# lh3/bfc

Measured on AMD Instinct MI355X. Metric: M k-mers/s counted (bloom+htab) on 150 bp reads, higher is better.
Workload: dtype u64

## Files before the change

bfc_amd/csrc/bfcg_bloom3.hip:

```cpp
#include <hip/hip_runtime.h>
#include <stdint.h>
#include <stdlib.h>
#include "kmer_dev.h"
#include "bfcg_internal.h"
#include "bfcg_dev.h"

using namespace bfcg;

#define B3_UND 0x40000000u
#define B3_SEEN16 0x8000u
#define B3_COLD_NR 8
#define B3_WALK_U 4
template <int BT, int PF, bool COLD>
__global__ __launch_bounds__(BT, PF <= 2 ? 8 : 6) void k_bloom3(KParams P, BloomArgs A)
{
	extern __shared__ __attribute__((aligned(16))) unsigned char smem[];
	__shared__ uint32_t s_list_n, s_ovf, s_pool_off, s_emit_n, s_fs_used, s_wb_n, s_pad3[2];
	const uint32_t f = blockIdx.x;
	const bool ho_log = A.ho_stride != 0;
	if (batch_poisoned(A)) { if (ho_log && threadIdx.x == 0) A.ho_mark[f] = A.ho_cur[f]; return; }
	uint32_t rs, n;
	region_list(A, f, rs, n);
	if (n == 0) { if (threadIdx.x == 0) { if (ho_log) A.ho_mark[f] = A.ho_cur[f]; else if (A.agg_cnt) A.agg_cnt[f] = 0; } return; }
	uint32_t ho_cur0 = 0;
	unsigned long long *ho_base;
	if (ho_log) {
		ho_cur0 = A.ho_cur[f];
		if (ho_cur0 + n > A.ho_stride) {
			if (threadIdx.x == 0) { atomicAdd(&A.stats[(size_t)(f & (ST_SLOTS - 1)) * ST_N + ST_ERR_POOL], 1ULL); A.ho_mark[f] = ho_cur0; }
			return;
		}
		ho_base = A.ho + (uint64_t)f * A.ho_stride + ho_cur0;
	} else ho_base = reinterpret_cast<unsigned long long *>(A.stream_out) + rs;
	A.stats += (size_t)(f & (ST_SLOTS - 1)) * ST_N;
	const uint32_t region_dw = 16u << P.R;
	unsigned char *sp = smem;
	unsigned int *region = reinterpret_cast<unsigned int *>(sp); sp += (size_t)region_dw * 4;
	const uint32_t nblk = 1u << P.R;
	unsigned int *bcnt = reinterpret_cast<unsigned int *>(sp), *boff = bcnt + nblk;
	if (COLD) sp += (size_t)(2 * nblk + 4) * 4;
	unsigned int *fs = reinterpret_cast<unsigned int *>(sp); if (!COLD) sp += (size_t)P.fs_cap * 4;
	unsigned int *la = reinterpret_cast<unsigned int *>(sp); sp += (size_t)P.list_cap * 4;
	unsigned int *lb = reinterpret_cast<unsigned int *>(sp); sp += (size_t)P.list_cap * 4;
	unsigned short *lc = reinterpret_cast<unsigned short *>(sp); sp += (size_t)P.list_cap * 2;
	unsigned short *ord = reinterpret_cast<unsigned short *>(sp);
	const uint32_t fs_mask = P.fs_cap - 1;
	const uint32_t *recs = A.recs + (uint64_t)rs * 3;
	unsigned int *g_region = reinterpret_cast<unsigned int *>(A.bloom) + (uint64_t)f * region_dw;
	const uint32_t imp = (P.f_base + f) >> P.F2;
	const Dec3 D = dec3_geom(P);
	const int tid = threadIdx.x, lane = tid & 63;
	const uint32_t mask_a = (1u << D.a) - 1u, imp_sh = D.n ? imp << D.lo : 0u, sh_up = D.lo + D.n;
#ifdef BFCG_MEASURE
	const bool timing = BFCG_ABL(P, 64) && tid == 0;
	long long tq[7] = {0, 0, 0, 0, 0, 0, 0};
	long long tc[7] = {0, 0, 0, 0, 0, 0, 0};
	if (timing) tq[0] = clock64();
#define B3_TC(i) do { if (timing) tc[i] = clock64(); } while (0)
#else
#define B3_TC(i) do { } while (0)
#endif
	auto addr3 = [&](uint32_t d0, uint32_t d1) -> uint32_t {
		const uint32_t y0d = d0 & mask_a, upper = y0d >> D.up;
		const uint32_t y0lo = D.n ? (y0d & D.lowmask) | imp_sh | (upper << sh_up) : y0d;
		const uint32_t y1lo = __builtin_amdgcn_alignbit(d1, d0, D.a) & D.mk32;
		const uint32_t hh = upper | (((y0lo - y1lo) ^ y1lo) << D.sh_x);
		uint32_t h2 = (hh >> 9) & 511u;
		h2 |= (uint32_t)((h2 & 31u) == 0);
		return (y0d & D.rmask) | ((hh & 511u) << 8) | (h2 << 17);
	};
	auto entry3 = [&](uint32_t d0, uint32_t d1) -> unsigned long long {
		const unsigned long long AA = d0 | ((unsigned long long)d1 << 32);
		const unsigned long long y1 = (AA >> D.a) & ((1ULL << P.k) - 1);
		const uint32_t y0d = d0 & mask_a;
		const unsigned long long id = (unsigned long long)((y0d & D.rmask) | ((y0d >> D.up) << D.R)) | (y1 << D.sh_y1);
		return (id << 1) | (unsigned long long)((d1 >> D.sh_flag) & 1u);
	};
	RecW<3> cur[PF], nxt[PF];
#pragma unroll
	for (int u = 0; u < PF; ++u) {
		const uint32_t i = tid + u * BT;
		cur[u].d[0] = cur[u].d[1] = cur[u].d[2] = 0; nxt[u] = cur[u];
		if (i < n) cur[u] = rec_load<3>(recs + (uint64_t)i * 3);
		if (i + BT * PF < n) nxt[u] = rec_load<3>(recs + (uint64_t)(i + BT * PF) * 3);
	}
	{
		const uint4 *src = reinterpret_cast<const uint4 *>(g_region);
		uint4 *dst = reinterpret_cast<uint4 *>(region);
		for (uint32_t i = tid; i < region_dw / 4; i += BT) dst[i] = src[i];
		if constexpr (COLD) { for (uint32_t i = tid; i < 2 * nblk + 4; i += BT) bcnt[i] = 0; }
		else {
			uint4 *f4 = reinterpret_cast<uint4 *>(fs);
			for (uint32_t i = tid; i < P.fs_cap / 4; i += BT) f4[i] = make_uint4(FS32_EMPTY, FS32_EMPTY, FS32_EMPTY, FS32_EMPTY);
		}
		if (tid == 0) { s_list_n = 0; s_emit_n = 0; s_ovf = 0; s_fs_used = 0; s_wb_n = 0; }
	}
	__syncthreads();
#ifdef BFCG_MEASURE
	if (timing) tq[1] = clock64();
#endif
	volatile uint32_t *v_ovf = &s_ovf;

	for (uint32_t base = 0; base < n; base += BT * PF) {
		uint32_t pk[PF], um[PF];
#pragma unroll
		for (int u = 0; u < PF; ++u) {
			pk[u] = 0; um[u] = 0;
			if (base + u * BT + (uint32_t)(tid & ~63) < n) {
				pk[u] = addr3(cur[u].d[0], cur[u].d[1]);
				const B3Pos b = b3_positions((pk[u] >> 8) & 511u, pk[u] >> 17);
				const uint32_t bl64 = (pk[u] & 255u) << 6;
				const uint32_t w0 = *b3_wordp(region, bl64, b.b0), w1 = *b3_wordp(region, bl64, b.b1), w2 = *b3_wordp(region, bl64, b.b2), w3 = *b3_wordp(region, bl64, b.b3);
				um[u] = (b3_bit(w0, b.b0) | (b3_bit(w1, b.b1) << 1) | (b3_bit(w2, b.b2) << 2) | (b3_bit(w3, b.b3) << 3)) ^ 15u;
			}
		}
		unsigned long long ms[PF], ml[PF];
		uint32_t tot_s = 0, tot_l = 0;
#pragma unroll
		for (int u = 0; u < PF; ++u) {
			const bool act = base + tid + u * BT < n;
			ms[u] = __ballot(act && um[u] == 0); ml[u] = __ballot(act && um[u] != 0);
			tot_s += (uint32_t)__popcll(ms[u]); tot_l += (uint32_t)__popcll(ml[u]);
		}
		uint32_t o_s = 0, o_l = 0;
		if (lane == 0) { if (tot_s) o_s = atomicAdd(&s_emit_n, tot_s); if (tot_l) o_l = atomicAdd(&s_list_n, tot_l); }
		o_s = __builtin_amdgcn_readfirstlane(o_s); o_l = __builtin_amdgcn_readfirstlane(o_l);
#pragma unroll
		for (int u = 0; u < PF; ++u) {
			const uint32_t below_lo = (uint32_t)__builtin_amdgcn_mbcnt_lo((uint32_t)ms[u], 0u), below_s = (uint32_t)__builtin_amdgcn_mbcnt_hi((uint32_t)(ms[u] >> 32), below_lo);
			const uint32_t blow_lo = (uint32_t)__builtin_amdgcn_mbcnt_lo((uint32_t)ml[u], 0u), below_l = (uint32_t)__builtin_amdgcn_mbcnt_hi((uint32_t)(ml[u] >> 32), blow_lo);
			const bool act = base + tid + u * BT < n;
			if (act && um[u] == 0) {
				ho_base[o_s + below_s] = entry3(cur[u].d[0], cur[u].d[1]);
				if (A.seen_out) A.seen_out[cur[u].d[2]] = 2;
			} else if (act) {
				const uint32_t li = o_l + below_l;
				if (li < P.list_cap) {
					la[li] = cur[u].d[2]; lb[li] = pk[u] | (um[u] << 26); lc[li] = (unsigned short)(base + tid + u * BT);
					if constexpr (COLD) __hip_atomic_fetch_add(&bcnt[pk[u] & 255u], 1u, __ATOMIC_RELAXED, __HIP_MEMORY_SCOPE_WORKGROUP);
				}
			}
			o_s += (uint32_t)__popcll(ms[u]); o_l += (uint32_t)__popcll(ml[u]);
// ... 590 lines not shown
```

bfc_amd/csrc/bfcg_ctx.hip:

```cpp
#include <hip/hip_runtime.h>
#include <stdint.h>
#include <stdio.h>
#include <stdlib.h>
#include <string.h>
#include <stdarg.h>
#include <sys/mman.h>
#include <time.h>
#include <vector>
#include <thread>
#include "bfc_gpu.h"
#include "bfcg_internal.h"
#include "bfc_host.h"
#include "kmer_dev.h"

using namespace bfcg;

static thread_local char g_err[512] = "";
enum { HO_MAX_PAGES = BFCG_HO_MAX_PAGES };
enum { OP_FLAG_WORDS = 12, OP_STICKY = 8 };
static double dbg_now(void) { struct timespec ts; clock_gettime(CLOCK_MONOTONIC, &ts); return ts.tv_sec + 1e-9 * ts.tv_nsec; }
static inline void set_seg_shift(KParams &P, int s, int blk_max) { P.seg_shift = s; P.seg_blk = s < blk_max ? s : blk_max; }
int bfcg::fail(const char *fmt, ...)
{
	va_list ap; va_start(ap, fmt); vsnprintf(g_err, sizeof(g_err), fmt, ap); va_end(ap);
// ... 4 lines not shown
struct bfcg_ctx {
	bfcg_params_t prm;
	KParams P;
	BatchBufs B;
	hipStream_t st;
	hipStream_t stA;
	hipStream_t stC;
	hipEvent_t evt[2][7];
	hipEvent_t evA[2], evB[2], evCopy;
	uint32_t *rows1[2], *chunk1[2], *start1[2]; uint64_t *recs1[2];
	uint8_t *d_seq2[2], *d_qual2[2];
	uint32_t *d_planes[2];
	uint64_t plane_cap;
	int cur, pend;
	int used[2];
	uint8_t *d_seq, *d_qual;
	unsigned long long *h_stats;
	unsigned long long *h_snap[2];
	uint64_t call_no, slot_call[2];
	int call_depth;
	uint64_t final_call, call_keys[64];
	uint64_t n_batches;
	float last_ms[6];
	double sum_ms[6]; uint64_t n_timed;
	int rw;
	uint64_t bloom_bytes;
	int n_ranks, rank, log2n;
	uint32_t *d_seg, *h_seg;
	size_t seg_words;
	uint64_t recv_cap;
	uint64_t keys_last, grow[2];
	uint64_t crowded_last;
	int stream_mode;
	uint32_t *stream_out; uint64_t n_stream_batches;
	double seen_per_pos;
	int cold;
	uint64_t seen_last, pos_final, slot_pos[2];
	int pipeline;
	int seg_ok;
	int seg_total_max;
	int seg_blk_max;
	int b3_ok;
	uint32_t fs_cap_w, list_cap_w;
	uint32_t list_cap_cw;
	uint32_t list_cap_c;
	int seg_init_shift;
	int seg_escaped;
	uint64_t n_seg_grow;
	int onepass_ok, onepass;
	uint32_t *op_cursor[2], *op_seg[2], *op_flags, *h_flags[2];
	int unfinished, unfinished_mg;
	uint32_t *h_rows[2]; int rows_slot;
	uint32_t op_cap; uint64_t op_min_pos;
	uint32_t *cnt2; uint32_t cap2; uint64_t recs2_n;
	struct opq_t { const uint8_t *seq, *qual; uint64_t n_pos; int slot; const void *recv; int mg; uint64_t call; } opq[4]; int n_opq;
	int mg_op2_ok, mg_op2, mg_op2_allowed; uint32_t *mg_seg[4];
	int mg_slab_ok; int mg_seg_slab[4];
	uint64_t n_replayed;
	int reused;
	int seg_no_grow;
	int seg_cap_shift;
	unsigned long long *ho, *ho_keys, *h_ho_keys[2]; uint32_t *ho_cur, *ho_mark; uint32_t ho_stride; int ho_K;
	int ho_pending;
	uint64_t ho_page_call[HO_MAX_PAGES];
	int slot_commit[2]; uint64_t slot_page_call[2][HO_MAX_PAGES];
	int slot_all_committed[2];
	uint64_t keys_known;
	int commit_absorbed;
	uint64_t keys_per_batch; int n_commits, ho_window;
	uint64_t n_seg_replayed, n_tab_replayed;
	uint64_t n_log_commits, max_commit_pages, n_to_legacy;
	unsigned long long *seg_spare; int seg_spare_shift;
};

extern "C" const char *bfcg_last_error(void) { return g_err; }
extern "C" void bfcg_set_error(const char *msg) { fail("%s", msg); }

extern "C" int bfcg_device_count(void)
{
	int ndev = 0;
	if (hipGetDeviceCount(&ndev) != hipSuccess) { (void)hipGetLastError(); return 0; }
	return ndev;
}

extern "C" void bfcg_params_default(bfcg_params_t *p)
{
	memset(p, 0, sizeof(*p));
	p->k = 33; p->q = 20; p->bf_shift = 33; p->n_hashes = 4; p->l_pre = 20;
	p->max_batch_pos = 1ULL << 27;
}

static int clamp_lpre(int k, int l_pre)
{
	if (k * 2 - l_pre > BFC_CH_KEYBITS) l_pre = k * 2 - BFC_CH_KEYBITS;
	if (l_pre > BFC_CH_MAXPRE) l_pre = BFC_CH_MAXPRE;
	return l_pre;
}

extern "C" bfcg_ctx_t *bfcg_create(const bfcg_params_t *prm)
{
	int ndev = 0;
	const bool timing = getenv("BFC_GPU_TIMING") != 0;
	const double t_c0 = dbg_now();
	if (hipGetDeviceCount(&ndev) != hipSuccess || ndev == 0) { fail("no HIP device available: the counting path has no CPU fallback"); return NULL; }
	const double t_c1 = dbg_now();
	if (prm->device < 0 || prm->device >= ndev) { fail("device %d out of range (%d devices)", prm->device, ndev); return NULL; }
// ... 70 lines not shown
			if (list > fs / 4 * 3) list = fs / 4 * 3;
			if (list > best_list) { best_list = list; best_fs = fs; }
		}
		fs = best_fs;
		if ((e = getenv("BFCG_FS")) != 0) { fs = (uint32_t)atoi(e); best_list = (uint32_t)((left - (size_t)fs * 4) / rwb); }
		P.fs_cap = fs;
		P.list_cap = best_list;
		if (P.list_cap > 8191) P.list_cap = 8191;
		c->fs_cap_w = c->list_cap_w = 0;
		if (P.b3 && !getenv("BFCG_LDS") && !(getenv("BFCG_B3_WARM") && atoi(getenv("BFCG_B3_WARM")) == 0)) {
			const size_t bw = 40900;
			if (bw > region + 16 + 8192) {
				const size_t lw = bw - region - 16;
				uint32_t fw = fs; while (fw > 1024 && (size_t)fw * 4 + (size_t)(P.list_cap / 4 * 3) * rwb > lw) fw >>= 1;
				uint32_t l = (size_t)fw * 4 < lw ? (uint32_t)((lw - (size_t)fw * 4) / rwb) : 0;
				if (l > P.list_cap) l = P.list_cap;
				if (l >= P.list_cap / 4 * 3 && fw >= 1024) { c->fs_cap_w = fw; c->list_cap_w = l; }
			}
		}
		c->list_cap_c = 0; c->list_cap_cw = 0;
		if (P.b3 && !(getenv("BFCG_B3_COLD") && atoi(getenv("BFCG_B3_COLD")) == 0)) {
			const size_t fixed = region + ((size_t)2 << P.R) * 4 + 16 + 16;
			if (budget > fixed + 12 * 256) {
				uint32_t l = (uint32_t)((budget - fixed) / 12);
				if (l > 4096) l = 4096;
				c->list_cap_c = l;
			}
			c->list_cap_cw = 0;
			if ((size_t)40900 > fixed + 12 * 256 && getenv("BFCG_B3_WALK_WARM") && atoi(getenv("BFCG_B3_WALK_WARM"))) c->list_cap_cw = (uint32_t)(((size_t)40900 - fixed) / 12);
		}
		P.b3fm = 0;
		if (prm->filter_mode && c->rw == 16 && bloom3fm_geometry_ok(P) && !getenv("BFCG_NO_B3")) {
			const size_t fixed = 2 * region + ((size_t)2 << P.R) * 4 + 16 + 16;
			if (budget > fixed + 10 * 256) {
				uint32_t l = (uint32_t)((budget - fixed) / 10);
				if ((e = getenv("BFCG_B3FM_LIST")) != 0 && atoi(e) >= 64 && (uint32_t)atoi(e) < l) l = (uint32_t)atoi(e);
				if (l > 4096) l = 4096;
				P.b3fm = 1; P.list_cap = l; P.fs_cap = 512;
			}
		}
		{
			const size_t room = (size_t)P.fs_cap * 4 + (size_t)P.list_cap * 8;
			uint32_t ct = 1; while ((size_t)ct * 2 * 8 <= room) ct <<= 1;
			P.ct_cap = ct;
		}
	}
	P.tab_cshift = prm->tab_cshift > 0 ? prm->tab_cshift : (P.l_pre <= 20 ? 5 : 3);
	if (prm->tab_cshift <= 0)
		while ((1ULL << (P.l_pre + P.tab_cshift)) < prm->max_batch_pos / 4 && P.l_pre + P.tab_cshift < 34) ++P.tab_cshift;
	P.track = (prm->track_order && !prm->filter_mode) ? 1 : 0;
	{ const char *e = getenv("BFCG_BT"); P.bloom_bt = e ? atoi(e) : (bloom_lds_bytes(P) > 80 * 1024 && !P.track && P.n_hashes == 4) ? 1024 : 512; if (P.bloom_bt != 1024 || P.track || P.n_hashes != 4) P.bloom_bt = 512; }
	c->n_ranks = n_ranks; c->rank = prm->rank; c->log2n = log2n;
	{ const char *e = getenv("BFCG_PIPELINE"); c->pipeline = e ? atoi(e) != 0 : prm->max_batch_pos <= (1ULL << 28); }

	if (n_ranks > 1 && log2n > P.F1) { fail("multi-GPU needs a two-level partition with 2^F1=%d >= n_ranks (bf_shift=%d is too small)", 1 << P.F1, P.bf_shift); bfcg_destroy(c); return NULL; }
	P.idx_rank = n_ranks > 1 ? (uint32_t)prm->rank << (32 - log2n) : 0u;
	c->bloom_bytes = (1ULL << (P.bf_shift - 3)) >> log2n;

	BatchBufs &B = c->B;
	B.max_kmers = prm->max_batch_pos;
	const int nb1 = 1 << P.F1, nfine = (1 << P.F) >> log2n;
	c->recv_cap = n_ranks > 1 ? B.max_kmers + B.max_kmers / 4 + (1u << 20) : B.max_kmers;
	BFCG_CKN(bfcg_destroy(c), hipStreamCreate(&c->st)); BFCG_CKN(bfcg_destroy(c), hipStreamCreate(&c->stA)); BFCG_CKN(bfcg_destroy(c), hipStreamCreate(&c->stC));
	for (int b = 0; b < 2; ++b) {
		for (int i = 0; i < 7; ++i) BFCG_CKN(bfcg_destroy(c), hipEventCreate(&c->evt[b][i]));
		BFCG_CKN(bfcg_destroy(c), hipEventCreateWithFlags(&c->evA[b], hipEventDisableTiming)); BFCG_CKN(bfcg_destroy(c), hipEventCreateWithFlags(&c->evB[b], hipEventDisableTiming));
	}
	BFCG_CKN(bfcg_destroy(c), hipEventCreateWithFlags(&c->evCopy, hipEventDisableTiming));
	{
		const uint64_t tile = (uint64_t)bfcg_tile_of_rw(c->rw / 4), tile1 = (uint64_t)bfcg_tile1_of_rw(c->rw / 4);
		const uint64_t tiles1 = (prm->max_batch_pos + tile1 - 1) / tile1, chunks1 = (tiles1 + BFCG_SCAN_CH - 1) / BFCG_SCAN_CH;
		const uint64_t rows2 = (c->recv_cap + c->recv_cap / 8) / tile + (uint64_t)nb1 * 16 + 8;
		for (int b = 0; b < 2; ++b) {
			BFCG_CKN(bfcg_destroy(c), hipMalloc(&c->rows1[b], sizeof(uint32_t) * tiles1 * nb1));
			BFCG_CKN(bfcg_destroy(c), hipMalloc(&c->chunk1[b], sizeof(uint32_t) * chunks1 * nb1));
			BFCG_CKN(bfcg_destroy(c), hipMalloc(&c->start1[b], sizeof(uint32_t) * (nb1 + 1) * 2));
		}
		B.rows1 = c->rows1[0]; B.chunk1 = c->chunk1[0]; B.start1 = c->start1[0]; B.row_base = B.start1 + nb1 + 1;
		if (P.F2 > 0) {
			BFCG_CKN(bfcg_destroy(c), hipMalloc(&B.rows2, sizeof(uint32_t) * rows2 * (1u << P.F2)));
			BFCG_CKN(bfcg_destroy(c), hipMalloc(&B.start2, sizeof(uint32_t) * (nfine + 1)));
		}
	}
	{
		const char *e = getenv("BFCG_ONEPASS");
		c->onepass_ok = n_ranks == 1 && P.F2 > 0 && !(e && atoi(e) == 0);
		uint64_t cap = (B.max_kmers + B.max_kmers / 8) / ((uint64_t)nb1 * 8) + 1;
		while (cap * nb1 * 8 > 0xffffffffULL) --cap;
		if (cap >= 1024) cap &= ~31ULL;
		else if (cap >= 8) cap &= ~3ULL;
		c->op_cap = (uint32_t)cap;
		c->op_min_pos = (e = getenv("BFCG_ONEPASS_MIN_TILES")) ? (uint64_t)atoi(e) * 4096 : (uint64_t)nb1 * 8 * 1024;
	}
	const uint64_t recs1_n = c->onepass_ok ? (uint64_t)c->op_cap * nb1 * 8 + (uint64_t)bfcg_tile1_of_rw(c->rw / 4) + 64 : B.max_kmers;
	BFCG_CKN(bfcg_destroy(c), hipMalloc(&c->recs1[0], recs1_n * c->rw));
	if (n_ranks == 1 && !c->pipeline) c->recs1[1] = c->recs1[0];
	else BFCG_CKN(bfcg_destroy(c), hipMalloc(&c->recs1[1], recs1_n * c->rw));
	{
		const char *e = getenv("BFCG_ONEPASS");
		c->mg_op2_ok = P.F2 > 0 && !(e && atoi(e) == 0);
	}
	{ const char *e = getenv("BFCG_MG_SLABS"); c->mg_slab_ok = P.F2 > 0 && !(e && atoi(e) == 0); }
	if (c->onepass_ok || c->mg_slab_ok) {
		for (int b = 0; b < 2; ++b) {
			BFCG_CKN(bfcg_destroy(c), hipMalloc(&c->op_cursor[b], sizeof(uint32_t) * (8 * nb1 * 32 + 32)));
			BFCG_CKN(bfcg_destroy(c), hipMalloc(&c->op_seg[b], sizeof(uint32_t) * ((size_t)25 * nb1 + 8)));
// ... 512 lines not shown
}


static KParams batch_params(const bfcg_ctx_t *c, int no_kstats, int onepass1)
{
	KParams Pt = c->P;
	Pt.no_kstats = no_kstats;
	Pt.dedupe = dedupe_hint(c);
	warm_tables(c, Pt);
	if (onepass1) {
		const char *e = getenv("BFCG_L2_BIG");
		const int want = e ? atoi(e) : 0;
		Pt.l2_big = c->cap2 && want > 0 && Pt.F2 >= (want == 1 ? 9 : 10) && scatter2_big_ok(Pt);
	}
	return Pt;
}

static int batch_bufs(bfcg_ctx_t *c, BatchBufs &Bt)
{
	if (ensure_agg(c) != 0 || use_stream(c) != 0) return -1;
	Bt = c->B;
	Bt.batch_hi = (unsigned long long)(c->n_batches + 1) << 32;
	Bt.stream = c->stream_mode; Bt.stream_out = c->stream_out;
	return 0;
}

struct StageB {
	const uint64_t *in1; const uint32_t *seg_beg, *seg_end; int n_seg, segs_per_bucket; const uint32_t *row_base, *bucket_start; uint64_t rec_bound;
	int slabs;
	int queued;
	uint64_t call, pos;
	const uint8_t *seq, *qual;
	const void *recv; const uint32_t *sizes; int sizes_slab;
	int finalise;
};

static int opq_push(bfcg_ctx_t *c, int b, const StageB &w)
{
	if (c->n_opq == 4) return fail("internal: one-pass queue overflow");
	int mg = 0;
	if (w.recv) {
		const size_t words = (size_t)c->n_ranks * (size_t)((1 << c->P.F1) >> c->log2n) * (w.sizes_slab ? 8 : 1);
		for (;; ++mg) { int used = 0; for (int i = 0; i < c->n_opq; ++i) used |= c->opq[i].mg == mg + 1; if (!used) break; }
		if (w.sizes) memcpy(c->mg_seg[mg], w.sizes, sizeof(uint32_t) * words); else memset(c->mg_seg[mg], 0, sizeof(uint32_t) * words);
		c->mg_seg_slab[mg++] = w.sizes_slab;
	}
	c->opq[c->n_opq++] = bfcg_ctx::opq_t{w.seq, w.qual, w.pos, b, w.recv, mg, w.call};
	return 0;
}

static int enqueue_stage_b(bfcg_ctx_t *c, int b, BatchBufs &Bt, const KParams &Pt, const StageB &w)
{
	if (handover_begin(c, Bt, b, w.slabs, w.call) != 0) return -1;
	run_stage_b(Pt, Bt, w.in1, w.seg_beg, w.seg_end, w.n_seg, w.segs_per_bucket, w.row_base, w.bucket_start, w.rec_bound, c->st, c->evt[b]);
	if (handover_end(c, Bt, b) != 0) return -1;
	if (w.queued) {
		BFCG_CK(hipMemcpyAsync(c->h_flags[b] + 1, c->op_flags + OP_STICKY, sizeof(uint32_t), hipMemcpyDeviceToHost, c->st));
		if (opq_push(c, b, w) != 0) return -1;
	}
	BFCG_CK(hipMemcpyAsync(c->h_snap[b], c->B.stats, sizeof(unsigned long long) * ST_N * (ST_SLOTS + 1), hipMemcpyDeviceToHost, c->st));
	c->slot_call[b] = c->call_no = w.call; c->slot_pos[b] = w.pos;
	BFCG_CK(hipEventRecord(c->evB[b], c->st));
	BFCG_CK(hipGetLastError());
	c->used[b] = 1;
	++c->n_batches;
	return w.finalise ? finalise_previous(c, b) : 0;
}

static int mg_stage_b(bfcg_ctx_t *c, int b, const void *d_recv, const uint32_t *d, int n_seg, int spb, uint64_t rec_bound, const uint32_t *sizes, int sizes_slab, int finalise)
{
	BatchBufs Bt;
	if (batch_bufs(c, Bt) != 0) return -1;
	const int op2_run = c->mg_op2 && c->mg_op2_allowed && c->cap2;
	const int op2 = op2_run && rec_bound >= 8 * nfine(c);
	if (op2_run) Bt.op_sticky = c->op_flags + OP_STICKY;
	if (op2) {
		Bt.cnt2 = c->cnt2; Bt.cap2 = c->cap2; Bt.op_flags = c->op_flags + 4 * b;
		BFCG_CK(hipMemsetAsync(Bt.op_flags, 0, 4 * sizeof(uint32_t), c->st));
	}
	const StageB w = {(const uint64_t *)d_recv, d, d + n_seg, n_seg, spb, d + 2 * n_seg, d + 3 * n_seg + 1, rec_bound, op2, op2_run, c->call_no + 1, rec_bound, nullptr, nullptr, d_recv, sizes, sizes_slab, finalise};
	return enqueue_stage_b(c, b, Bt, batch_params(c, 0, 0), w);
}


extern "C" int bfcg_mg_info(bfcg_ctx_t *c, int out[4])
{
	out[0] = 1 << c->P.F1; out[1] = (1 << c->P.F1) >> c->log2n; out[2] = c->rw; out[3] = c->n_ranks;
	return 0;
}

static int mg_scatter2(bfcg_ctx_t *c, const uint8_t *d_seq, const uint8_t *d_qual, uint64_t n_pos, void *d_send, uint32_t *counts, int no_kstats);
extern "C" int bfcg_mg_scatter(bfcg_ctx_t *c, const uint8_t *d_seq, const uint8_t *d_qual, uint64_t n_pos, void *d_send, uint32_t *counts) { return mg_scatter2(c, d_seq, d_qual, n_pos, d_send, counts, 0); }
int bfcg::mg_scatter_again(bfcg_ctx_t *c, const uint8_t *d_seq, const uint8_t *d_qual, uint64_t n_pos, void *d_send, uint32_t *counts) { return mg_scatter2(c, d_seq, d_qual, n_pos, d_send, counts, 1); }
static inline hipStream_t mg_stage_a_stream(bfcg_ctx_t *c) { return c->n_ranks == 1 && !c->pipeline ? c->st : c->stA; }
static int mg_stage_a_begin(bfcg_ctx_t *c, int b, hipStream_t sA, const uint8_t *d_seq, const uint8_t **d_qual, uint64_t n_pos)
{
	if (batch_fits(c, n_pos) != 0) return -1;
	BFCG_CK(hipSetDevice(c->prm.device));
	if (n_pos == 0) {
		for (int i = 0; i < 3; ++i) BFCG_CK(hipEventRecord(c->evt[b][i], sA));
		return 1;
	}
	return same_block_offset(c, b, d_seq, d_qual, n_pos, sA);
}
static BatchBufs mg_slab_bufs(const bfcg_ctx_t *c, int b, uint32_t own_delta)
{
// ... 676 lines not shown
```

bfc_amd/csrc/bfcg_dev.h:

```cpp
#pragma once
#include <hip/hip_runtime.h>
#include <stdint.h>
#include "kmer_dev.h"
#include "bfcg_internal.h"

using namespace bfcg;

template <int RD> struct RecW { uint32_t d[RD]; };

template <int RD> __device__ __forceinline__ RecW<RD> rec_load(const uint32_t *p);
template <> __device__ __forceinline__ RecW<3> rec_load<3>(const uint32_t *p)
{ const uint3 v = *reinterpret_cast<const uint3 *>(p); RecW<3> r; r.d[0] = v.x; r.d[1] = v.y; r.d[2] = v.z; return r; }
template <> __device__ __forceinline__ RecW<4> rec_load<4>(const uint32_t *p)
{ const uint4 v = *reinterpret_cast<const uint4 *>(p); RecW<4> r; r.d[0] = v.x; r.d[1] = v.y; r.d[2] = v.z; r.d[3] = v.w; return r; }
template <> __device__ __forceinline__ RecW<5> rec_load<5>(const uint32_t *p)
{ RecW<5> r; r.d[0] = p[0]; r.d[1] = p[1]; r.d[2] = p[2]; r.d[3] = p[3]; r.d[4] = p[4]; return r; }
template <int RD> __device__ __forceinline__ void rec_store(uint32_t *p, const RecW<RD> &r);
template <> __device__ __forceinline__ void rec_store<3>(uint32_t *p, const RecW<3> &r)
{ *reinterpret_cast<uint3 *>(p) = make_uint3(r.d[0], r.d[1], r.d[2]); }
template <> __device__ __forceinline__ void rec_store<4>(uint32_t *p, const RecW<4> &r)
{ *reinterpret_cast<uint4 *>(p) = make_uint4(r.d[0], r.d[1], r.d[2], r.d[3]); }
template <> __device__ __forceinline__ void rec_store<5>(uint32_t *p, const RecW<5> &r)
{ p[0] = r.d[0]; p[1] = r.d[1]; p[2] = r.d[2]; p[3] = r.d[3]; p[4] = r.d[4]; }

// ... 9 lines not shown

#define FS_EMPTY 0xffffffffffffffffULL

template <bool GLOBAL>
__device__ __forceinline__ bool fs_insert(unsigned long long *tab, uint32_t cap_mask, uint32_t bitoff, uint32_t idx, uint32_t max_probe)
{
	const unsigned long long e = ((unsigned long long)bitoff << 32) | idx;
	uint32_t p = ((bitoff * 0x9E3779B1u) >> 12 ^ bitoff) & cap_mask;
	for (uint32_t probe = 0; probe <= max_probe; ++probe, p = (p + 1) & cap_mask) {
		unsigned long long cur = GLOBAL ? __hip_atomic_load(&tab[p], __ATOMIC_RELAXED, __HIP_MEMORY_SCOPE_AGENT) : tab[p];
		if (cur == FS_EMPTY) {
			cur = atomicCAS(&tab[p], FS_EMPTY, e);
			if (cur == FS_EMPTY) return true;
		}
		if ((uint32_t)(cur >> 32) == bitoff) { if (e < cur) atomicMin(&tab[p], e); return true; }
	}
	return false;
}
template <bool GLOBAL>
__device__ __forceinline__ bool fs_lookup(const unsigned long long *tab, uint32_t cap_mask, uint32_t bitoff, uint32_t &first)
{
	uint32_t p = ((bitoff * 0x9E3779B1u) >> 12 ^ bitoff) & cap_mask;
	for (uint32_t probe = 0; probe <= cap_mask; ++probe, p = (p + 1) & cap_mask) {
		unsigned long long cur = GLOBAL ? __hip_atomic_load((unsigned long long *)&tab[p], __ATOMIC_RELAXED, __HIP_MEMORY_SCOPE_AGENT) : tab[p];
		if (cur == FS_EMPTY) return false;
		if ((uint32_t)(cur >> 32) == bitoff) { first = (uint32_t)cur; return true; }
	}
	return false;
}

struct BloomArgs {
	const uint32_t *recs;
	const uint32_t *start;
	unsigned long long *bloom;
	unsigned long long *bloom_hi;
	unsigned long long *table;
	unsigned long long *stats;
	uint64_t *tab_ovf; uint32_t tab_ovf_cap; unsigned long long *ovf_cnt;
	unsigned long long *pool; uint32_t pool_slices;
	uint8_t *seen_out;
	uint64_t *agg_out;
	uint32_t *agg_cnt;
	uint32_t *stream_out;
	unsigned long long *seg_tab;
	uint32_t n_fine;
	TabOrder ord;
	unsigned long long batch_hi;
	const uint32_t *cnt2; uint32_t cap2;
	unsigned long long *ho; uint32_t ho_stride; uint32_t *ho_cur; uint32_t *ho_mark;
	uint32_t ho_pages, ho_mark_stride;
	unsigned long long *ho_keys;
	const uint32_t *flags;
	const uint32_t *sticky;
};

__device__ __forceinline__ void region_list(const BloomArgs &A, uint32_t f, uint32_t &rs, uint32_t &n)
{
	if (A.cap2) { const uint32_t c = A.cnt2[f]; rs = f * A.cap2; n = c < A.cap2 ? c : A.cap2; }
	else if (A.cnt2) { rs = A.start[f]; n = A.cnt2[f]; }
	else { rs = A.start[f]; n = A.start[f + 1] - rs; }
}
__device__ __forceinline__ bool batch_poisoned(const BloomArgs &A) { return (A.sticky && *A.sticky) || (A.flags && (A.flags[0] | A.flags[2])); }


struct Dec3 { int ok, a, lo, n, up, sh_x, R, sh_flag, sh_y1; uint32_t lowmask, rmask, mk32; };
__device__ __forceinline__ Dec3 dec3_geom(const KParams &P)
{
	Dec3 g;
	g.a = P.k - P.rec_n; g.lo = P.rec_lo; g.n = P.rec_n; g.up = P.rec_n ? P.rec_lo : P.bf_shift - 9; g.sh_x = P.k - (P.bf_shift - 9);
	g.R = P.R; g.sh_flag = g.a + P.k - 32; g.sh_y1 = P.k - P.F;
	g.lowmask = P.rec_n ? (1u << (P.rec_lo & 31)) - 1u : 0xffffffffu; g.rmask = (1u << P.R) - 1u; g.mk32 = P.k >= 32 ? 0xffffffffu : (1u << P.k) - 1u;
	g.ok = P.k >= P.bf_shift - 9 && P.bf_shift + 9 <= 2 * P.k && g.a >= 1 && g.a <= 31 && g.a + P.k >= 32 && (P.rec_n == 0 || P.rec_lo + P.rec_n <= 31)
	       && g.up <= g.a && g.sh_x >= 0 && g.sh_x <= 31 && g.sh_y1 >= 0 && g.sh_y1 <= 32 && (P.rec_n == 0 || P.rec_lo + P.rec_n == P.bf_shift - 9) && P.R <= g.up;
	return g;
}

#define FS32_EMPTY 0xffffffffu
__device__ __forceinline__ uint32_t fs32_slot(uint32_t bitoff, uint32_t mask) { return ((bitoff * 0x9E3779B1u) >> 12 ^ bitoff) & mask; }

__device__ __forceinline__ bool fs32_insert(unsigned int *fs, uint32_t mask, uint32_t bitoff, uint32_t li, uint32_t idx, const unsigned int *list_idx)
{
	const uint32_t e = (bitoff << 13) | li;
	uint32_t p = fs32_slot(bitoff, mask);
	for (int probe = 0; probe < 1024; ++probe, p = (p + 1) & mask) {
		uint32_t cur = fs[p];
		if (cur == FS32_EMPTY) {
			cur = atomicCAS(&fs[p], FS32_EMPTY, e);
			if (cur == FS32_EMPTY) return true;
		}
		if ((cur >> 13) == bitoff) {
			while (list_idx[cur & 0x1fffu] > idx) {
				uint32_t old = atomicCAS(&fs[p], cur, e);
				if (old == cur) break;
				cur = old;
			}
			return true;
		}
	}
	return false;
}
__device__ __forceinline__ bool fs32_compete(unsigned int *fs, uint32_t mask, uint32_t bitoff, uint32_t li, uint32_t idx, const unsigned int *list_idx)
{
	const uint32_t e = (bitoff << 13) | li;
	uint32_t p = fs32_slot(bitoff, mask);
	for (uint32_t probe = 0; probe <= mask; ++probe, p = (p + 1) & mask) {
		uint32_t cur = fs[p];
// ... 51 lines not shown
```

bfc_amd/csrc/bfcg_internal.h:

```cpp
#pragma once
#include <hip/hip_runtime.h>
#define BFCG_TILE1 4096
#define BFCG_BT1 256
#define BFCG_SCAN_CH 64
static inline int bfcg_rec_dwords(int k, int rec_n) { const int bits = 2 * k - rec_n + 33; return bits <= 96 ? 3 : bits <= 128 ? 4 : 5; }
static constexpr int bfcg_tile_of_rw(int rw) { return rw == 5 ? 2048 : rw == 4 ? 3072 : 4096; }
static constexpr int bfcg_tile1_of_rw(int rw) { return rw == 3 ? 4096 : 3072; }
#define BFCG_MAXB 1024
#define BFCG_HO_MAX_PAGES 8
#ifdef BFCG_MEASURE
#define BFCG_ABL(P, bits) ((P).ablate & (bits))
#else
#define BFCG_ABL(P, bits) 0
#endif
#include <stdint.h>
struct bfcg_ctx; struct bfcg_kcov;

extern "C" void bfcg_set_error(const char *msg);
extern "C" void *bfcg_bloom_slice(struct bfcg_ctx *c, int which, uint64_t *bytes);
extern "C" int bfcg_resident_register(const void *bf, void *dev, int device, int n_shift);

#define BFCG_UT_NBUF 20
struct bfcg_kmers {
	int k, l_pre, cshift, device, owns_table;
// ... 17 lines not shown
	uint64_t n_keys; int has_keys;
	float last_ms;
};

namespace bfcg {
#define BFCG_LOCAL __attribute__((visibility("hidden")))

enum { ST_KMERS = 0, ST_HIGH, ST_SEEN, ST_KEYS, ST_TAB_OVF, ST_ERR_POOL, ST_SLOW_BUCKETS, ST_CROWDED , ST_N = 16 };
enum { ST_SLOTS = 256 };

struct KParams {
	int k, q, bf_shift, n_hashes, l_pre, filter_mode;
	int R;
	int F, F1, F2;
	int tab_cshift;
	uint32_t fs_cap, list_cap;
	uint32_t ag_cap;
	uint32_t idx_rank;
	int track;
	int ablate;
	int bloom_bt;
	int seg;
	int seg_shift;
	int seg_blk;
	int seg_lo, seg_hi;
	uint32_t f_base;
	int no_kstats;
	int dedupe;
	uint32_t ct_cap;
	int rec_lo, rec_n;
	int b3;
	int b3_warm;
	int b3fm;
	int l2_big;
	int b3_cold;
};

struct BatchBufs {
	uint32_t *rows1, *chunk1;
	uint32_t *start1, *row_base;
	uint32_t *rows2, *start2;
	uint64_t *recs1, *recs2;
	uint64_t max_kmers;
	unsigned long long *bloom, *bloom_hi, *table;
	unsigned long long *stats;
	uint64_t *tab_ovf; uint32_t tab_ovf_cap;
	unsigned long long *pool; uint32_t pool_slices;
	uint8_t *seen_out;
	uint64_t *agg_out; uint32_t *agg_cnt;
	uint32_t *stream_out; int stream;
	uint32_t *op_cursor, *op_flags, *op_sticky, *op_seg; uint32_t op_cap;
	uint32_t op_own_lo, op_own_n, op_own_delta;
	uint32_t *cnt2; uint32_t cap2;
	uint32_t *cnt_live;
	unsigned long long *ho; uint32_t ho_stride; uint32_t *ho_cur, *ho_mark; uint32_t ho_mark_stride, ho_page; int ho_commit; unsigned long long *ho_keys;
	unsigned long long *seg_tab;
	unsigned long long *tab_first, *sub_last;
	unsigned long long batch_hi;
};

void run_stage_a(const KParams &P, const BatchBufs &B, const uint8_t *seq, const uint8_t *qual, int64_t n_pos, uint64_t *out1, hipStream_t st, hipEvent_t *ev);
void run_stage_a_onepass(const KParams &P, const BatchBufs &B, const uint8_t *seq, const uint8_t *qual, int64_t n_pos, uint64_t *out1, hipStream_t st, hipEvent_t *ev);
void run_stage_b(const KParams &P, const BatchBufs &B, const uint64_t *in1, const uint32_t *seg_beg, const uint32_t *seg_end, int n_seg, int segs_per_bucket,
                 const uint32_t *row_base, const uint32_t *bucket_start, uint64_t n_rec_bound, hipStream_t st, hipEvent_t *ev);
void run_pack_rows(const KParams &P, const BatchBufs &B, int n_ranks, uint32_t row_w, uint32_t *rows, hipStream_t st);
void run_seg_setup_mg(const KParams &P, int rw_dwords, const uint32_t *rows, uint32_t row_w, int n_ranks, int s_lo, int s_hi, uint32_t cap, uint32_t *seg, unsigned long long *total, hipStream_t st);
void run_batch(const KParams &P, const BatchBufs &B, const uint8_t *seq, const uint8_t *qual, int64_t n_pos, hipStream_t st, hipEvent_t *ev);
int bloom_lds_bytes(const KParams &P);
bool bloom3fm_geometry_ok(const KParams &P);
bool bloom3_geometry_ok(const KParams &P);
BFCG_LOCAL bool scatter2_big_ok(const KParams &P);
hipError_t set_bloom_lds_attr(const KParams &P);
void run_query(const KParams &P, const uint8_t *seq, int64_t n_pos, const void *bloom, uint8_t *flags, hipStream_t st);
void run_kcov(const KParams &P, const uint8_t *seq, int64_t n_pos, int min_occ, const void *tab, uint8_t *flags, uint16_t *out, hipStream_t st);
void run_streak(int k, float min_frac, const uint8_t *flags, const uint64_t *off, uint64_t n_reads, int32_t *out_start, int32_t *out_end, hipStream_t st);
void run_hash_only(const KParams &P, const uint8_t *seq, const uint8_t *qual, int64_t n_pos, uint64_t *out, hipStream_t st);
void run_table_replay(const KParams &P, unsigned long long *tab, const uint64_t *src, uint64_t n, unsigned long long *stats, uint64_t *ovf, uint32_t ovf_cap,
                      unsigned long long *first, unsigned long long *sub_last, hipStream_t st);
void run_seg_rehash(const KParams &P, const unsigned long long *old_tab, int old_shift, int old_blk, unsigned long long *new_tab, uint32_t n_fine, hipStream_t st);
void run_seg_replay(const KParams &P, unsigned long long *seg_tab, const uint64_t *src, uint64_t n, unsigned long long *stats, uint64_t *ovf, uint32_t ovf_cap, hipStream_t st);
void run_seg_to_table(const KParams &P, const unsigned long long *seg_tab, uint32_t n_fine, unsigned long long *tab, unsigned long long *stats, uint64_t *ovf, uint32_t ovf_cap, hipStream_t st);
hipError_t set_seg_lds_attr(void);
hipError_t set_scatter1wc_lds_attr(void);
void run_commit_pages(const KParams &P, const BatchBufs &B, uint32_t n_fine, uint32_t pages, hipStream_t st);
#define BFCG_SEG_MAX_SHIFT 14
#define BFCG_SEG_TOTAL_MAX 24
void run_table_rehash(const KParams &P, const unsigned long long *old_tab, int cshift_old, unsigned long long *new_tab,
                      const unsigned long long *old_first, unsigned long long *new_first, hipStream_t st);

BFCG_LOCAL int fail(const char *fmt, ...) __attribute__((format(printf, 1, 2)));
#define BFCG_CK(call) do { hipError_t e_ = (call); if (e_ != hipSuccess) return bfcg::fail("%s failed: %s (%s:%d)", #call, hipGetErrorString(e_), __FILE__, __LINE__); } while (0)
#define BFCG_CKN(cleanup, call) do { hipError_t e_ = (call); if (e_ != hipSuccess) { bfcg::fail("%s failed: %s (%s:%d)", #call, hipGetErrorString(e_), __FILE__, __LINE__); cleanup; (void)hipGetLastError(); return NULL; } } while (0)

static inline int is_acgt(uint8_t ch) { ch &= 0xDF; return ch == 'A' || ch == 'C' || ch == 'G' || ch == 'T'; }

struct resident_t { const void *host; void *dev; int device, n_shift, k, l_pre, cshift; };
BFCG_LOCAL int resident_put(const resident_t &r);
BFCG_LOCAL void *resident_take(const void *host, int device, int n_shift, int k, int l_pre, int cshift);

const unsigned long long *ctx_borrow_table(::bfcg_ctx *c, KParams *P, int *device);
int ctx_table_k(::bfcg_ctx *c);
BFCG_LOCAL int mg_scatter_again(::bfcg_ctx *c, const uint8_t *d_seq, const uint8_t *d_qual, uint64_t n_pos, void *d_send, uint32_t *counts);
BFCG_LOCAL int mg_slab_info(::bfcg_ctx *c, uint32_t out[2]);
BFCG_LOCAL int mg_scatter_slabs(::bfcg_ctx *c, const uint8_t *d_seq, const uint8_t *d_qual, uint64_t n_pos, void *d_send, uint32_t own_delta, uint32_t *fills, int *overflow);
BFCG_LOCAL int mg_row_words(::bfcg_ctx *c);
BFCG_LOCAL int mg_async_ok(::bfcg_ctx *c);
// ... 25 lines not shown
```

bfc_amd/csrc/bfcg_kernels.hip:

```cpp
#include <hip/hip_runtime.h>
#include <stdint.h>
#include <stdlib.h>
#include <string.h>
#include <stdio.h>
#include "kmer_dev.h"
#include "bfcg_internal.h"
#include "bfcg_dev.h"
#include "bfcg_k1.h"

using namespace bfcg;

#define WAVE 64








template <typename W> __device__ __forceinline__ uint32_t fine_id(const KParams &P, uint64_t y0, uint64_t y1)
{
	W m = kmask<W>(P.k);
	uint64_t hash = bloom_hash<W>(P.k, (W)y0, (W)y1, m);
// ... 1939 lines not shown
	static const bool force2d = getenv("BFCG_SEG_GRID2D") != nullptr;
	if (wgs * bt < (1ULL << 32) && !force2d) return dim3((unsigned)wgs, 1u);
	return dim3(n_fine, 1u << ub);
}
static void launch_commit_seg(const KParams &P, const BloomArgs &A, int nfine, hipStream_t st)
{
	const BloomK k = commit_seg_kernel(P.seg_blk);
	hipLaunchKernelGGL(k.fn, seg_grid(P, (uint32_t)nfine, (uint32_t)k.bt), dim3(k.bt), commit_seg_lds_bytes(P.seg_blk), st, P, A);
	dbg_sync(st, "k_commit_seg");
}
void run_commit_pages(const KParams &P, const BatchBufs &B, uint32_t n_fine, uint32_t pages, hipStream_t st)
{
	BloomArgs A;
	memset(&A, 0, sizeof(A));
	A.stats = B.stats; A.tab_ovf = B.tab_ovf; A.tab_ovf_cap = B.tab_ovf_cap; A.ovf_cnt = B.stats + (size_t)ST_SLOTS * ST_N; A.seg_tab = B.seg_tab; A.n_fine = n_fine;
	A.ho = B.ho; A.ho_stride = B.ho_stride; A.ho_cur = B.ho_cur; A.ho_mark = B.ho_mark; A.ho_mark_stride = B.ho_mark_stride; A.ho_pages = pages; A.ho_keys = B.ho_keys;
	launch_commit_seg(P, A, (int)n_fine, st);
}

template <typename W, int RW>
static std::pair<const uint32_t *, const uint32_t *> run_level2_t(const KParams &P, const BatchBufs &B, const uint32_t *in1, const uint32_t *seg_beg, const uint32_t *seg_end, int n_seg,
                                                                  int segs_per_bucket, const uint32_t *row_base, const uint32_t *bucket_start, uint64_t n_rec_bound, hipStream_t st)
{
	if (P.F2 == 0) return {in1, bucket_start};
	const int nb_loc = n_seg / segs_per_bucket, nfine = nb_loc << P.F2;
	int v = S2V_TWO_PASS;
	if (B.cap2) {
		const bool fast = (RW == 3 || RW == 4) && scatter2_fast(P);
		v = !fast ? S2V_ONEPASS : RW == 3 && P.l2_big ? S2V_FAST_BIG : S2V_FAST;
		hipMemsetAsync(B.cnt2, 0, sizeof(uint32_t) * (size_t)nfine, st);
	} else {
		hipLaunchKernelGGL((k_hist2<W, RW, bfcg_tile_of_rw(RW), BT2>), dim3(level2_grid(n_rec_bound, bfcg_tile_of_rw(RW), n_seg)), dim3(BT2), 0, st, P, in1, seg_beg, seg_end, n_seg, segs_per_bucket, row_base, B.rows2);
		hipLaunchKernelGGL(k_scan2, dim3(nb_loc), dim3((1 << P.F2) < 64 ? 64 : (1 << P.F2)), 0, st, P, bucket_start, segs_per_bucket, row_base, B.rows2, B.start2, B.cnt_live);
	}
	const Scatter2K k = scatter2_kernel<W, RW>(v);
	hipLaunchKernelGGL(have(k.fn, "k_scatter2", v, RW), dim3(level2_grid(n_rec_bound, k.tile, n_seg)), dim3(k.bt), scatter2_lds_bytes(RW, k.tile, 1 << P.F2), st, P, in1, seg_beg, seg_end, n_seg, segs_per_bucket, row_base,
	                   B.cap2 ? nullptr : B.rows2, (uint32_t *)B.recs2, B.cap2 ? OnePass2{B.cnt2, B.cap2, B.op_flags} : OnePass2{nullptr, 0u, nullptr});
	dbg_sync(st, "level 2");
	return {(const uint32_t *)B.recs2, B.start2};
}

template <typename W, int RW>
static BloomArgs run_bloom_t(const KParams &P, const BatchBufs &B, const uint32_t *fine_recs, const uint32_t *fine_start, int nfine, hipStream_t st)
{
	BloomArgs A;
	memset(&A, 0, sizeof(A));
	A.recs = fine_recs; A.start = fine_start; A.bloom = B.bloom; A.bloom_hi = B.bloom_hi; A.table = B.table; A.stats = B.stats;
	A.tab_ovf = B.tab_ovf; A.tab_ovf_cap = B.tab_ovf_cap; A.ovf_cnt = B.stats + (size_t)ST_SLOTS * ST_N; A.pool = B.pool; A.pool_slices = B.pool_slices; A.seen_out = B.seen_out;
	A.agg_out = B.agg_out; A.agg_cnt = B.agg_cnt; A.n_fine = (uint32_t)nfine; A.stream_out = nullptr; A.seg_tab = nullptr;
	A.ord.first = B.tab_first; A.ord.sub_last = B.sub_last; A.batch_hi = B.batch_hi;
	A.cnt2 = nullptr; A.cap2 = 0; A.flags = B.op_flags; A.sticky = B.op_sticky;
	if (P.F2 > 0 && B.cap2) { A.cnt2 = B.cnt2; A.cap2 = B.cap2; }
	else if (P.F2 > 0 && B.cnt_live) A.cnt2 = B.cnt_live;
	const bool h4 = P.n_hashes == 4;
	if (P.filter_mode && B.bloom_hi) {
		if (RW == 4 && P.b3fm) run_bloom3fm(P, A, nfine, (size_t)bloom_lds_bytes(P), st);
		else launch_bloom<W, RW>(!h4 ? BV_FM_ANYH : P.bloom_bt == 1024 ? BV_FM_1024 : BV_FM, P, A, nfine, st);
	} else if (P.seg && B.seg_tab && (B.stream_out || B.ho)) {
		A.stream_out = B.stream_out; A.seg_tab = B.seg_tab; A.table = nullptr; A.agg_out = nullptr;
		A.ho = B.ho; A.ho_stride = B.ho_stride; A.ho_cur = B.ho_cur; A.ho_mark = B.ho_stride ? B.ho_mark + (size_t)B.ho_page * B.ho_mark_stride : nullptr;
		if (RW == 3 && P.b3 && (P.b3_cold || !P.dedupe)) run_bloom3(P, A, nfine, (size_t)bloom_lds_bytes(P), st);
		else launch_bloom<W, RW>(!h4 ? BV_SEG_ANYH : RW == 3 && bloom_fast3(P) ? BV_SEG_F3 : BV_SEG, P, A, nfine, st);
	} else if (B.stream && B.stream_out && !P.track && h4) {
		A.stream_out = B.stream_out;
		launch_bloom<W, RW>(BV_STREAM, P, A, nfine, st);
	} else if (P.track) launch_bloom<W, RW>(h4 ? BV_TRACK : BV_TRACK_ANYH, P, A, nfine, st);
	else launch_bloom<W, RW>(!h4 ? BV_ANYH : P.bloom_bt == 1024 ? BV_1024 : BV_512, P, A, nfine, st);
	return A;
}

template <typename W, int RW>
static void run_commit_t(const KParams &P, const BatchBufs &B, BloomArgs &A, int nfine, hipStream_t st)
{
	const auto waves = [&] { return dim3((unsigned)((nfine + 4 * COMMIT_RPW - 1) / (4 * COMMIT_RPW))); };
	if (A.seg_tab) {
		if (B.ho_stride == 0 || B.ho_commit) {
			A.ho_mark = B.ho_mark; A.ho_mark_stride = B.ho_mark_stride; A.ho_pages = B.ho_page + 1; A.ho_keys = B.ho_keys;
			launch_commit_seg(P, A, nfine, st);
		}
	} else if (A.stream_out) hipLaunchKernelGGL((k_commit_stream<W, RW>), waves(), dim3(256), 0, st, P, A);
	else if (B.agg_out && nfine > (1 << 18)) hipLaunchKernelGGL((P.track ? k_commit<W, true, true> : k_commit<W, false, true>), waves(), dim3(256), 0, st, P, A);
	else if (B.agg_out) hipLaunchKernelGGL((P.track ? k_commit<W, true, false> : k_commit<W, false, false>), dim3((unsigned)(((uint64_t)nfine * P.ag_cap + 255) / 256)), dim3(256), 0, st, P, A);
}

template <typename W, int RW>
static void run_stage_b_t(const KParams &P, const BatchBufs &B, const uint32_t *in1, const uint32_t *seg_beg, const uint32_t *seg_end, int n_seg,
                          int segs_per_bucket, const uint32_t *row_base, const uint32_t *bucket_start, uint64_t n_rec_bound, hipStream_t st, hipEvent_t *ev)
{
	const int nfine = (n_seg / segs_per_bucket) << P.F2;
	const auto [fine_recs, fine_start] = run_level2_t<W, RW>(P, B, in1, seg_beg, seg_end, n_seg, segs_per_bucket, row_base, bucket_start, n_rec_bound, st);
	if (ev) hipEventRecord(ev[3], st);
	BloomArgs A = run_bloom_t<W, RW>(P, B, fine_recs, fine_start, nfine, st);
	if (ev) hipEventRecord(ev[4], st);
	if (A.seg_tab || A.stream_out) dbg_sync(st, "k_bloom");
	run_commit_t<W, RW>(P, B, A, nfine, st);
	if (A.flags) hipLaunchKernelGGL(k_seal, dim3(1), dim3(1), 0, st, B.op_flags, B.op_sticky);
	if (ev) hipEventRecord(ev[5], st);
}

#define DISPATCH_W(fn, ...) do { const int rw_ = bfcg_rec_dwords(P.k, P.rec_n); \
	if (P.k <= 32) { if (rw_ == 3) fn<uint32_t, 3>(__VA_ARGS__); else fn<uint32_t, 4>(__VA_ARGS__); } \
	else if (rw_ == 3) fn<uint64_t, 3>(__VA_ARGS__); else if (rw_ == 4) fn<uint64_t, 4>(__VA_ARGS__); else fn<uint64_t, 5>(__VA_ARGS__); } while (0)

void run_stage_a(const KParams &P, const BatchBufs &B, const uint8_t *seq, const uint8_t *qual, int64_t n_pos, uint64_t *out1, hipStream_t st, hipEvent_t *ev)
{ DISPATCH_W(run_stage_a_t, P, B, seq, qual, n_pos, (uint32_t *)out1, st, ev); }

// ... 119 lines not shown
```

Measured before the change: 41430.

## Issue bloom region, control words and first records eagerly at kernel entry

At the top of the bloom3 kernel, an 'eager' mode now issues the global loads for the bloom region slice (into registers), the poison flags, counts, ho cursor and, when one-pass cap2 layout is used, the first record batch, all at once. These loads no longer wait serially on one another, so the dependent-load latency at kernel start overlaps. The region is then written to LDS from registers. This costs extra registers (up to 1024/BT uint4 per thread) and some loads wasted on poisoned or empty blocks. The mode is enabled by default when the batch holds at least 16 positions per fine bucket.

```diff
diff --git a/bfc_amd/csrc/bfcg_bloom3.hip b/bfc_amd/csrc/bfcg_bloom3.hip
--- a/bfc_amd/csrc/bfcg_bloom3.hip
+++ b/bfc_amd/csrc/bfcg_bloom3.hip
@@ -18,14 +18,43 @@
 	__shared__ uint32_t s_list_n, s_ovf, s_pool_off, s_emit_n, s_fs_used, s_wb_n, s_pad3[2];
 	const uint32_t f = blockIdx.x;
 	const bool ho_log = A.ho_stride != 0;
-	if (batch_poisoned(A)) { if (ho_log && threadIdx.x == 0) A.ho_mark[f] = A.ho_cur[f]; return; }
+#ifdef BFCG_MEASURE
+	const long long t_start = clock64();
+#endif
+	const bool eager = A.eager != 0, spec = eager && A.cap2 != 0;
+	constexpr int B3_SL = 1024 / BT;
+	uint4 sl[B3_SL];
+	uint32_t e_st = 0, e_f0 = 0, e_f2 = 0, e_c = 0, e_s = 0, e_h = 0;
+	RecW<3> cur[PF], nxt[PF];
+#pragma unroll
+	for (int u = 0; u < PF; ++u) { cur[u].d[0] = cur[u].d[1] = cur[u].d[2] = 0; nxt[u] = cur[u]; }
+#pragma unroll
+	for (int j = 0; j < B3_SL; ++j) sl[j] = make_uint4(0, 0, 0, 0);
+	if (eager) {
+		const uint4 *src = reinterpret_cast<const uint4 *>(reinterpret_cast<const unsigned int *>(A.bloom) + (uint64_t)f * (16u << P.R));
+#pragma unroll
+		for (int j = 0; j < B3_SL; ++j) if ((uint32_t)(threadIdx.x + j * BT) < (4u << P.R)) sl[j] = src[threadIdx.x + j * BT];
+		const uint32_t *const any = reinterpret_cast<const uint32_t *>(A.stats);
+		const uint32_t *const p_st = A.sticky ? A.sticky : any, *const p_fl = A.flags ? A.flags : any;
+		const uint32_t *const p_c = A.cnt2 ? A.cnt2 + f : A.start + f + 1, *const p_s = A.cap2 ? any : A.start + f, *const p_h = ho_log ? A.ho_cur + f : any;
+		e_st = *p_st; e_f0 = p_fl[0]; e_f2 = p_fl[2]; e_c = *p_c; e_s = *p_s; e_h = *p_h;
+		if (spec) {
+			const uint32_t *r0 = A.recs + (uint64_t)(f * A.cap2) * 3;
+#pragma unroll
+			for (int u = 0; u < PF; ++u) { const uint32_t i = threadIdx.x + u * BT; if (i < A.cap2) cur[u] = rec_load<3>(r0 + (uint64_t)i * 3); }
+		}
+	}
+	const bool poisoned = eager ? (((A.sticky ? e_st : 0u) | (A.flags ? e_f0 | e_f2 : 0u)) != 0u) : batch_poisoned(A);
+	if (poisoned) { if (ho_log && threadIdx.x == 0) A.ho_mark[f] = A.ho_cur[f]; return; }
 	uint32_t rs, n;
-	region_list(A, f, rs, n);
+	if (!eager) region_list(A, f, rs, n);
+	else if (A.cap2) { rs = f * A.cap2; n = e_c < A.cap2 ? e_c : A.cap2; }
+	else { rs = e_s; n = A.cnt2 ? e_c : e_c - e_s; }
 	if (n == 0) { if (threadIdx.x == 0) { if (ho_log) A.ho_mark[f] = A.ho_cur[f]; else if (A.agg_cnt) A.agg_cnt[f] = 0; } return; }
 	uint32_t ho_cur0 = 0;
 	unsigned long long *ho_base;
 	if (ho_log) {
-		ho_cur0 = A.ho_cur[f];
+		ho_cur0 = eager ? e_h : A.ho_cur[f];
 		if (ho_cur0 + n > A.ho_stride) {
 			if (threadIdx.x == 0) { atomicAdd(&A.stats[(size_t)(f & (ST_SLOTS - 1)) * ST_N + ST_ERR_POOL], 1ULL); A.ho_mark[f] = ho_cur0; }
 			return;
@@ -55,7 +84,7 @@
 	const bool timing = BFCG_ABL(P, 64) && tid == 0;
 	long long tq[7] = {0, 0, 0, 0, 0, 0, 0};
 	long long tc[7] = {0, 0, 0, 0, 0, 0, 0};
-	if (timing) tq[0] = clock64();
+	if (timing) tq[0] = t_start;
 #define B3_TC(i) do { if (timing) tc[i] = clock64(); } while (0)
 #else
 #define B3_TC(i) do { } while (0)
@@ -76,18 +105,23 @@
 		const unsigned long long id = (unsigned long long)((y0d & D.rmask) | ((y0d >> D.up) << D.R)) | (y1 << D.sh_y1);
 		return (id << 1) | (unsigned long long)((d1 >> D.sh_flag) & 1u);
 	};
-	RecW<3> cur[PF], nxt[PF];
 #pragma unroll
 	for (int u = 0; u < PF; ++u) {
 		const uint32_t i = tid + u * BT;
-		cur[u].d[0] = cur[u].d[1] = cur[u].d[2] = 0; nxt[u] = cur[u];
-		if (i < n) cur[u] = rec_load<3>(recs + (uint64_t)i * 3);
+		if (!spec && i < n) cur[u] = rec_load<3>(recs + (uint64_t)i * 3);
 		if (i + BT * PF < n) nxt[u] = rec_load<3>(recs + (uint64_t)(i + BT * PF) * 3);
+	}
+	if (spec) {
+#pragma unroll
+		for (int u = 0; u < PF; ++u) if ((uint32_t)(tid + u * BT) >= n) cur[u].d[0] = cur[u].d[1] = cur[u].d[2] = 0;
 	}
 	{
 		const uint4 *src = reinterpret_cast<const uint4 *>(g_region);
 		uint4 *dst = reinterpret_cast<uint4 *>(region);
-		for (uint32_t i = tid; i < region_dw / 4; i += BT) dst[i] = src[i];
+		if (eager) {
+#pragma unroll
+			for (int j = 0; j < B3_SL; ++j) if ((uint32_t)(tid + j * BT) < region_dw / 4) dst[tid + j * BT] = sl[j];
+		} else for (uint32_t i = tid; i < region_dw / 4; i += BT) dst[i] = src[i];
 		if constexpr (COLD) { for (uint32_t i = tid; i < 2 * nblk + 4; i += BT) bcnt[i] = 0; }
 		else {
 			uint4 *f4 = reinterpret_cast<uint4 *>(fs);
diff --git a/bfc_amd/csrc/bfcg_ctx.hip b/bfc_amd/csrc/bfcg_ctx.hip
--- a/bfc_amd/csrc/bfcg_ctx.hip
+++ b/bfc_amd/csrc/bfcg_ctx.hip
@@ -80,6 +80,7 @@
 	int unfinished, unfinished_mg;
 	uint32_t *h_rows[2]; int rows_slot;
 	uint32_t op_cap; uint64_t op_min_pos;
+	int eager;
 	uint32_t *cnt2; uint32_t cap2; uint64_t recs2_n;
 	struct opq_t { const uint8_t *seq, *qual; uint64_t n_pos; int slot; const void *recv; int mg; uint64_t call; } opq[4]; int n_opq;
 	int mg_op2_ok, mg_op2, mg_op2_allowed; uint32_t *mg_seg[4];
@@ -256,6 +257,7 @@
 	{ const char *e = getenv("BFCG_BT"); P.bloom_bt = e ? atoi(e) : (bloom_lds_bytes(P) > 80 * 1024 && !P.track && P.n_hashes == 4) ? 1024 : 512; if (P.bloom_bt != 1024 || P.track || P.n_hashes != 4) P.bloom_bt = 512; }
 	c->n_ranks = n_ranks; c->rank = prm->rank; c->log2n = log2n;
 	{ const char *e = getenv("BFCG_PIPELINE"); c->pipeline = e ? atoi(e) != 0 : prm->max_batch_pos <= (1ULL << 28); }
+	{ const char *e = getenv("BFCG_EAGER"); c->eager = e ? atoi(e) != 0 : -1; }
 
 	if (n_ranks > 1 && log2n > P.F1) { fail("multi-GPU needs a two-level partition with 2^F1=%d >= n_ranks (bf_shift=%d is too small)", 1 << P.F1, P.bf_shift); bfcg_destroy(c); return NULL; }
 	P.idx_rank = n_ranks > 1 ? (uint32_t)prm->rank << (32 - log2n) : 0u;
@@ -874,6 +876,7 @@
 static int enqueue_stage_b(bfcg_ctx_t *c, int b, BatchBufs &Bt, const KParams &Pt, const StageB &w)
 {
 	if (handover_begin(c, Bt, b, w.slabs, w.call) != 0) return -1;
+	Bt.eager = c->eager >= 0 ? c->eager : w.pos >= (uint64_t)16 * nfine(c);
 	run_stage_b(Pt, Bt, w.in1, w.seg_beg, w.seg_end, w.n_seg, w.segs_per_bucket, w.row_base, w.bucket_start, w.rec_bound, c->st, c->evt[b]);
 	if (handover_end(c, Bt, b) != 0) return -1;
 	if (w.queued) {
diff --git a/bfc_amd/csrc/bfcg_dev.h b/bfc_amd/csrc/bfcg_dev.h
--- a/bfc_amd/csrc/bfcg_dev.h
+++ b/bfc_amd/csrc/bfcg_dev.h
@@ -85,6 +85,7 @@
 	unsigned long long *ho_keys;
 	const uint32_t *flags;
 	const uint32_t *sticky;
+	uint32_t eager;
 };
 
 __device__ __forceinline__ void region_list(const BloomArgs &A, uint32_t f, uint32_t &rs, uint32_t &n)
diff --git a/bfc_amd/csrc/bfcg_internal.h b/bfc_amd/csrc/bfcg_internal.h
--- a/bfc_amd/csrc/bfcg_internal.h
+++ b/bfc_amd/csrc/bfcg_internal.h
@@ -93,6 +93,7 @@
 	uint32_t *op_cursor, *op_flags, *op_sticky, *op_seg; uint32_t op_cap;
 	uint32_t op_own_lo, op_own_n, op_own_delta;
 	uint32_t *cnt2; uint32_t cap2;
+	int eager;
 	uint32_t *cnt_live;
 	unsigned long long *ho; uint32_t ho_stride; uint32_t *ho_cur, *ho_mark; uint32_t ho_mark_stride, ho_page; int ho_commit; unsigned long long *ho_keys;
 	unsigned long long *seg_tab;
diff --git a/bfc_amd/csrc/bfcg_kernels.hip b/bfc_amd/csrc/bfcg_kernels.hip
--- a/bfc_amd/csrc/bfcg_kernels.hip
+++ b/bfc_amd/csrc/bfcg_kernels.hip
@@ -2015,6 +2015,7 @@
 	A.cnt2 = nullptr; A.cap2 = 0; A.flags = B.op_flags; A.sticky = B.op_sticky;
 	if (P.F2 > 0 && B.cap2) { A.cnt2 = B.cnt2; A.cap2 = B.cap2; }
 	else if (P.F2 > 0 && B.cnt_live) A.cnt2 = B.cnt_live;
+	A.eager = B.eager != 0;
 	const bool h4 = P.n_hashes == 4;
 	if (P.filter_mode && B.bloom_hi) {
 		if (RW == 4 && P.b3fm) run_bloom3fm(P, A, nfine, (size_t)bloom_lds_bytes(P), st);
```

Result: faster. 42670 (median of 6 runs) (+3.0%).
